# ambonvik/cimba

Measured on NVIDIA H100. Metric: M/M/1 simulated events/sec (FEL pops/s), higher is better.
Workload: dtype f64

## Files before the change

cimba_b200/csrc/mm1_fast.cuh:

```cuda
#pragma once

#include "engine.cuh"
#include "queue_model.cuh"
#include "rng.cuh"

namespace cimba_b200 {

#ifndef MM1_PARK_MASK
#define MM1_PARK_MASK 7u
#endif
#ifndef MM1_COLD_BATCH
#define MM1_COLD_BATCH 4
#endif

__device__ __forceinline__ void sts_f64(uint32_t addr, double v)
{
    asm volatile("st.shared.f64 [%0], %1;" :: "r"(addr), "d"(v) : "memory");
}

__device__ __forceinline__ double lds_f64(uint32_t addr)
{
    double v;
    asm volatile("ld.shared.f64 %0, [%1];" : "=d"(v) : "r"(addr) : "memory");
    return v;
}

__device__ __forceinline__ uint32_t pack_key(uint32_t counter, uint32_t action)
{
    return (counter << 2) | action;
}

template <bool TRACE>
__global__ void __launch_bounds__(QUEUE_BLOCK)
mm1_kernel(const QueueArgs a)
{
    __shared__ double exp_x[256];
    __shared__ double ring_smem[QUEUE_WINDOW * QUEUE_BLOCK];

    for (unsigned i = threadIdx.x; i < 256u; i += blockDim.x) {
        exp_x[i] = zig::zig_exp_x[i];
    }
    __syncthreads();

    constexpr unsigned FULL = 0xffffffffu;
    constexpr uint32_t WMASK = QUEUE_WINDOW - 1;
    constexpr uint32_t ROW = QUEUE_BLOCK * 8u;
    const double INF = __longlong_as_double(0x7ff0000000000000LL);
    const unsigned lane = threadIdx.x & 31u;
    const uint64_t gtid = (uint64_t)blockIdx.x * blockDim.x + threadIdx.x;
    uint64_t trial;
    bool alive;
    if (a.mapping == 32) {
        trial = gtid >> 5;
        alive = (lane == 0u) && (trial < a.num_trials);
    }
    else {
        trial = gtid;
        alive = trial < a.num_trials;
    }

    Sfc64 rng;
    rng.a = rng.b = rng.c = rng.d = 0u;
    double t_arr = INF, t_srv = INF;
    uint32_t k_arr = 0u, k_srv = 0u;
    uint32_t issued = 0u;
    double now = 0.0, stamp = 0.0, sum_wait = 0.0;
    double arr_mean = 1.0, srv_mean = 1.0;
    uint32_t produced = 0u, served = 0u, dropped = 0u, status = TRIAL_OK, longest = 0u;
    const uint32_t quota = (uint32_t)a.num_objects;
    uint32_t win = (uint32_t)__cvta_generic_to_shared(&ring_smem[threadIdx.x]);
    uint32_t tab = (uint32_t)__cvta_generic_to_shared(&exp_x[0]);
    __shared__ double scratch_smem[QUEUE_BLOCK];
    uint32_t scratch = (uint32_t)__cvta_generic_to_shared(&scratch_smem[threadIdx.x]);
    asm volatile("" : "+r"(win), "+r"(tab), "+r"(scratch));
    double *const spill = (a.spill_cap && alive) ? a.spill + trial * a.spill_cap : nullptr;
    const uint32_t spill_mask = a.spill_cap - 1u;

    uint64_t u_next = 0u;
    double e_next = 0.0;
    uint32_t pops = 0u;

    if (alive) {
        arr_mean = a.arr_mean[trial];
        srv_mean = a.srv_mean[trial];
        rng.seed(fmix64(a.master_seed, a.first_trial + trial));
        t_arr = 0.0; k_arr = pack_key(1u, ACT_START);
        t_srv = 0.0; k_srv = pack_key(2u, ACT_START);
        issued = 2u;
        u_next = rng.next();
        e_next = __dmul_rn(lds_f64(tab + ((uint32_t)u_next & 0xffu) * 8u), __ull2double_rn(u_next));
    }

    uint32_t flags = alive ? 1u : 0u;
    uint32_t step = 0u;

    while (__any_sync(FULL, flags & 1u)) {
        const bool go0 = (flags & 3u) == 1u;
        const bool first_arr = (t_arr < t_srv) | ((t_arr == t_srv) & (k_arr < k_srv));
        const uint32_t key = first_arr ? k_arr : k_srv;
        const uint32_t act = key & 3u;
        const bool go = go0 & (key != 0u);
        const bool done = go0 & (key == 0u);
        const bool is_arr = go & first_arr;
        const bool is_srv = go & !first_arr;
        const bool wake = act == ACT_WAKE_TIME;
        if (TRACE) {
            if (go && pops < a.trace_cap) {
                a.trace_key[trial * a.trace_cap + pops] = key >> 2;
                a.trace_time[trial * a.trace_cap + pops] = first_arr ? t_arr : t_srv;
            }
            pops += go ? 1u : 0u;
        }
        if (go) now = first_arr ? t_arr : t_srv;

        const uint32_t q_len = produced - served;
        const bool put = is_arr & wake;
        const bool put_far = put & (q_len >= (uint32_t)QUEUE_WINDOW);
        sts_f64((put & !put_far) ? win + (produced & WMASK) * ROW : scratch, now);
        if (put_far) {
            if (spill != nullptr && q_len - QUEUE_WINDOW <= spill_mask) {
                spill[produced & spill_mask] = now;
            }
            else {
                status |= TRIAL_ERR_QUEUE_OVERFLOW;
                dropped++;
                served++;
            }
        }
        if (put) produced++;
        longest = max(longest, produced - served);
        const bool ring_bell = put & (k_srv == 0u);
        if (ring_bell) {
            issued++;
            t_srv = now;
            k_srv = pack_key(issued, ACT_WAKE_RESOURCE);
        }

        const bool finished = is_srv & wake;
        const double new_sum = __dadd_rn(sum_wait, __dsub_rn(now, stamp));
        if (finished) sum_wait = new_sum;
        const bool take = is_srv & (produced != served);
        const uint32_t head_slot = win + (served & WMASK) * ROW;
        const double head_stamp = lds_f64(head_slot);
        if (take) stamp = head_stamp;
        if (take & (produced - served > (uint32_t)QUEUE_WINDOW)) {
            sts_f64(head_slot, spill[(served + QUEUE_WINDOW) & spill_mask]);
        }
        if (take) served++;

        const bool draw = take | (is_arr & (produced < quota));
        const bool hot = Sfc64::exp_is_hot(u_next);
        const bool push = draw & hot;
        const double when = __dadd_rn(now, __dmul_rn(is_arr ? arr_mean : srv_mean, e_next));
        if (push) issued++;
        const double t_new = push ? when : INF;
        const uint32_t k_new = push ? pack_key(issued, ACT_WAKE_TIME) : 0u;
        if (is_arr) { t_arr = t_new; k_arr = k_new; }
        if (is_srv) { t_srv = t_new; k_srv = k_new; }
        if (draw & !hot) flags = is_arr ? 7u : 3u;
        if (push) {
            u_next = rng.next();
            e_next = __dmul_rn(lds_f64(tab + ((uint32_t)u_next & 0xffu) * 8u), __ull2double_rn(u_next));
        }

        if (done) {
            flags = 0u;
            if (a.events)    a.events[trial] = issued;
            if (a.objects)   a.objects[trial] = served - dropped;
            if (a.t_end)     a.t_end[trial] = now;
            if (a.sum_wait)  a.sum_wait[trial] = sum_wait;
            if (a.status)    a.status[trial] = status | (issued > 0x3ffffff0u ? TRIAL_ERR_KEY_OVERFLOW : 0u);
            if (a.max_queue) a.max_queue[trial] = longest;
        }
        if ((++step & MM1_PARK_MASK) != 0u) {
            continue;
        }
        const unsigned pm = __ballot_sync(FULL, flags & 2u);
        if (pm != 0u) {
            const unsigned am = __ballot_sync(FULL, flags & 1u);
            if (__popc(pm) >= MM1_COLD_BATCH || pm == am) {
                if (flags & 2u) {
                    const bool parked_is_arr = (flags & 4u) != 0u;
                    const double mean = parked_is_arr ? arr_mean : srv_mean;
                    const double at = __dadd_rn(now, __dmul_rn(mean, rng.exp_cold(u_next)));
                    issued++;
                    if (parked_is_arr) { t_arr = at; k_arr = pack_key(issued, ACT_WAKE_TIME); }
                    else               { t_srv = at; k_srv = pack_key(issued, ACT_WAKE_TIME); }
                    flags = 1u;
                    u_next = rng.next();
                    e_next = __dmul_rn(lds_f64(tab + ((uint32_t)u_next & 0xffu) * 8u), __ull2double_rn(u_next));
                }
            }
        }
    }
    if (a.diag != nullptr && lane == 0u) {
        atomicAdd(a.diag, (unsigned long long)step);
        atomicAdd(a.diag + 1, 1ull);
    }
}

}
```

cimba_b200/csrc/rng.cuh:

```cuda
#pragma once

#include <cstdint>
#ifndef CMB_HOST_BUILD
#include <cuda_runtime.h>
#endif

#include "glibc_exp.cuh"
#include "zig_tables.cuh"

namespace cimba_b200 {

__host__ __device__ __forceinline__ uint64_t fmix64(uint64_t seed, uint64_t nonce)
{
    uint64_t h = seed + nonce;
    h ^= h >> 33;
    h *= 0xff51afd7ed558ccdULL;
    h ^= h >> 33;
    h *= 0xc4ceb9fe1a85ec53ULL;
    h ^= h >> 33;
    return h;
}

struct ZigHot {
    double exp_x[256];
    double nor_x[256];
};

__device__ __forceinline__ void stage_zig_hot(ZigHot &hot, bool want_normal)
{
    for (unsigned i = threadIdx.x; i < 256u; i += blockDim.x) {
        hot.exp_x[i] = zig::zig_exp_x[i];
        hot.nor_x[i] = want_normal ? zig::zig_nor_x[i] : 0.0;
    }
}

__device__ __noinline__ double zig_exp(double x)
{
    return glibc_exp(x);
}

constexpr double TWO_POW_64 = 18446744073709551616.0;
constexpr double TWO_POW_63 = 9223372036854775808.0;
constexpr double TWO_POW_M53 = 1.1102230246251565404e-16;

struct Sfc64 {
    uint64_t a, b, c, d;

    __device__ __forceinline__ uint64_t next()
    {
        const uint64_t out = a + b + d++;
        a = b ^ (b >> 11);
#if !defined(SFC64_NO_IMAD) && !defined(CMB_HOST_BUILD)
        {
            uint32_t lo, hi;
            asm("mov.b64 {%0, %1}, %2;" : "=r"(lo), "=r"(hi) : "l"(c));
            uint64_t w;
            asm("mul.wide.u32 %0, %1, 9;" : "=l"(w) : "r"(lo));
            uint32_t wl, wh;
            asm("mov.b64 {%0, %1}, %2;" : "=r"(wl), "=r"(wh) : "l"(w));
            asm("mad.lo.u32 %0, %1, 9, %2;" : "=r"(wh) : "r"(hi), "r"(wh));
            asm("mov.b64 %0, {%1, %2};" : "=l"(b) : "r"(wl), "r"(wh));
        }
#else
        b = c + (c << 3);
#endif
        c = ((c << 24) | (c >> 40)) + out;
        return out;
    }

    __device__ __forceinline__ void rewind()
    {
        const uint64_t pc = b * 0x8e38e38e38e38e39ULL;
        uint64_t pb = a;
        pb ^= pb >> 11;
        pb ^= pb >> 22;
        pb ^= pb >> 44;
        const uint64_t out = c - ((pc << 24) | (pc >> 40));
        d -= 1u;
        a = out - pb - d;
        b = pb;
        c = pc;
    }

    __device__ __forceinline__ void seed(uint64_t s)
    {
        uint64_t w[4];
#pragma unroll
        for (int i = 0; i < 4; i++) {
            uint64_t z = (s += 0x9e3779b97f4a7c15ULL);
            z = (z ^ (z >> 30)) * 0xbf58476d1ce4e5b9ULL;
            z = (z ^ (z >> 27)) * 0x94d049bb133111ebULL;
            w[i] = z ^ (z >> 31);
        }
        a = w[0];
        b = w[1];
        c = w[2];
        d = w[3];
#pragma unroll 1
        for (int i = 0; i < 20; i++) {
            (void)next();
        }
    }

    __device__ __forceinline__ double uniform01()
    {
        return __dmul_rn(__ull2double_rn(next() >> 11), TWO_POW_M53);
    }

    __device__ __forceinline__ double uniform(double lo, double hi)
    {
        return __dadd_rn(lo, __dmul_rn(__dsub_rn(hi, lo), uniform01()));
    }

    __device__ __forceinline__ unsigned bernoulli(double p)
    {
        return uniform01() <= p ? 1u : 0u;
    }

    __device__ __forceinline__ long long dice(long long lo, long long hi)
    {
        const double x = __dmul_rn(__ll2double_rn(hi - lo + 1), uniform01());
        return (long long)floor(__dadd_rn(__ll2double_rn(lo), x));
    }


    static __device__ __forceinline__ bool exp_is_hot(uint64_t u)
    {
        return (unsigned)(u & 0xffu) <= ZIG_EXP_MAX;
    }

    static __device__ __forceinline__ double exp_hot(const ZigHot &hot, uint64_t u)
    {
        return __dmul_rn(hot.exp_x[u & 0xffu], __ull2double_rn(u));
    }

    __device__ __forceinline__ double exp_cold(uint64_t ux)
    {
        double shift = 0.0;
        for (;;) {
            uint64_t uy = next();
            unsigned j = (unsigned)(uy & 0xffu);
            if (next() >= zig::zig_exp_prob[j]) {
                j = zig::zig_exp_alias[j];
            }
            if (j > 0u) {
                const double xj = zig::zig_exp_x[j];
                const double dx = __dsub_rn(zig::zig_exp_x[j - 1u], xj);
                for (;;) {
                    if (uy > (UINT64_MAX - ux)) {
                        uy = UINT64_MAX - uy;
                        ux = UINT64_MAX - ux;
                    }
                    const uint64_t gap = (UINT64_MAX - ux) - uy;
                    const double x = __dadd_rn(__dmul_rn(xj, TWO_POW_64),
                                               __dmul_rn(dx, __ull2double_rn(ux)));
                    if (gap >= zig::zig_exp_concavity[j]) {
                        return __dadd_rn(x, shift);
                    }
                    const double y0 = zig::zig_exp_y[j - 1u];
                    const double y = __dadd_rn(__dmul_rn(y0, TWO_POW_64),
                                               __dmul_rn(__dsub_rn(zig::zig_exp_y[j], y0),
                                                         __ull2double_rn(uy)));
                    if (y <= zig_exp(-x)) {
                        return __dadd_rn(x, shift);
                    }
                    uy = next();
                    ux = next();
                }
            }
            shift = __dadd_rn(shift, ZIG_EXP_TAIL);
            ux = next();
            const unsigned i = (unsigned)(ux & 0xffu);
            if (i <= ZIG_EXP_MAX) {
                return __dadd_rn(__dmul_rn(zig::zig_exp_x[i], __ull2double_rn(ux)), shift);
            }
        }
    }

    __device__ __forceinline__ double std_exponential(const ZigHot &hot)
    {
        const uint64_t u = next();
        return exp_is_hot(u) ? exp_hot(hot, u) : exp_cold(u);
    }

    __device__ __forceinline__ double std_exponential_global()
    {
        const uint64_t u = next();
        return exp_is_hot(u) ? __dmul_rn(zig::zig_exp_x[u & 0xffu], __ull2double_rn(u)) : exp_cold(u);
    }

    __device__ __forceinline__ double exponential(const ZigHot &hot, double mean)
    {
        return __dmul_rn(mean, std_exponential(hot));
    }

    __device__ __forceinline__ double erlang(const ZigHot &hot, unsigned k, double m)
    {
        double x = 0.0;
        for (unsigned i = 0u; i < k; i++) {
            x = __dadd_rn(x, exponential(hot, m));
        }
        return x;
    }


    __device__ __forceinline__ int64_t draw63()
    {
        return (int64_t)(next() & (uint64_t)INT64_MAX);
    }

    static __device__ __forceinline__ double nor_x_of(unsigned j, int64_t ix)
    {
        const double xj = zig::zig_nor_x[j];
        return __dadd_rn(__dmul_rn(xj, TWO_POW_63),
                         __dmul_rn(__dsub_rn(zig::zig_nor_x[j - 1u], xj), __ll2double_rn(ix)));
    }

    static __device__ __forceinline__ double nor_y_of(unsigned j, int64_t iy)
    {
        const double y0 = zig::zig_nor_y[j - 1u];
        return __dadd_rn(__dmul_rn(y0, TWO_POW_63),
                         __dmul_rn(__dsub_rn(zig::zig_nor_y[j], y0),
                                   __ull2double_rn((uint64_t)iy)));
    }

    static __device__ __forceinline__ double nor_pdf_scaled(double x)
    {
        return zig_exp(__dmul_rn(__dmul_rn(-0.5, x), x));
    }

    __device__ __forceinline__ double nor_cold(const ZigHot &hot, int64_t ix)
    {
        const double sign = (ix < 0) ? -1.0 : 1.0;
        ix &= INT64_MAX;
        int64_t iy = draw63();
        unsigned j = (unsigned)(iy & 0xff);
        if (ix >= zig::zig_nor_prob[j]) {
            j = zig::zig_nor_alias[j];
        }
        if (j > ZIG_NOR_INFLECTION) {
            for (;;) {
                const double x = nor_x_of(j, ix);
                const int64_t gap = (INT64_MAX - ix) - iy;
                if (gap >= 0) {
                    return __dmul_rn(sign, x);
                }
                if (gap + zig::zig_nor_convexity[j] >= 0) {
                    if (nor_y_of(j, iy) < nor_pdf_scaled(x)) {
                        return __dmul_rn(sign, x);
                    }
                }
                ix = draw63();
                iy = draw63();
            }
        }
        else if (j == 0u) {
            double x, z;
            do {
                x = __dmul_rn(ZIG_NOR_INV_TAIL, exponential(hot, 1.0));
                z = exponential(hot, 1.0);
            } while (__dmul_rn(2.0, z) <= __dmul_rn(x, x));
            return __dmul_rn(sign, __dadd_rn(x, ZIG_NOR_TAIL));
        }
        else if (j < ZIG_NOR_INFLECTION) {
            for (;;) {
                if (iy > INT64_MAX - ix) {
                    iy = INT64_MAX - iy;
                    ix = INT64_MAX - ix;
                }
                const double x = nor_x_of(j, ix);
                const int64_t gap = (INT64_MAX - ix) - iy;
                if (gap >= zig::zig_nor_concavity[j]) {
                    return __dmul_rn(sign, x);
                }
                if (nor_y_of(j, iy) <= nor_pdf_scaled(x)) {
                    return __dmul_rn(sign, x);
                }
                ix = draw63();
                iy = draw63();
            }
        }
        else {
            for (;;) {
                const double x = nor_x_of(j, ix);
                const int64_t gap = (INT64_MAX - ix) - iy;
                if (gap >= zig::zig_nor_concavity[j]) {
                    return __dmul_rn(sign, x);
                }
                if (gap + zig::zig_nor_convexity[j] > 0) {
                    if (nor_y_of(j, iy) < nor_pdf_scaled(x)) {
                        return __dmul_rn(sign, x);
                    }
                }
                ix = draw63();
                iy = draw63();
            }
        }
    }

    __device__ __forceinline__ double std_normal(const ZigHot &hot)
    {
        const int64_t ix = (int64_t)next();
        const unsigned i = (unsigned)(ix & 0xff);
        return (i <= ZIG_NOR_MAX) ? __dmul_rn(hot.nor_x[i], __ll2double_rn(ix))
                                  : nor_cold(hot, ix);
    }

    __device__ __forceinline__ double normal(const ZigHot &hot, double mu, double sigma)
    {
        return __dadd_rn(mu, __dmul_rn(sigma, std_normal(hot)));
    }
};

}
```

Measured before the change: 132.3 billion.

## Unroll two events per warp-vote iteration and route RNG shifts through IMAD

```diff
diff --git a/cimba_b200/csrc/mm1_fast.cuh b/cimba_b200/csrc/mm1_fast.cuh
--- a/cimba_b200/csrc/mm1_fast.cuh
+++ b/cimba_b200/csrc/mm1_fast.cuh
@@ -11,6 +11,9 @@
 #endif
 #ifndef MM1_COLD_BATCH
 #define MM1_COLD_BATCH 4
+#endif
+#ifndef MM1_STEPS
+#define MM1_STEPS 2
 #endif
 
 __device__ __forceinline__ void sts_f64(uint32_t addr, double v)
@@ -78,7 +81,13 @@
 
     uint64_t u_next = 0u;
     double e_next = 0.0;
+    uint32_t off_next = 0u;
     uint32_t pops = 0u;
+    const auto refill = [&]() {
+        u_next = rng.next_imad();
+        off_next = imad_hi(imad_lo((uint32_t)u_next, IMAD_K2P24, 0u), IMAD_K2P11, 0u);
+        e_next = __dmul_rn(lds_f64(tab + off_next), __ull2double_rn(u_next));
+    };
 
     if (alive) {
         arr_mean = a.arr_mean[trial];
@@ -87,23 +96,21 @@
         t_arr = 0.0; k_arr = pack_key(1u, ACT_START);
         t_srv = 0.0; k_srv = pack_key(2u, ACT_START);
         issued = 2u;
-        u_next = rng.next();
-        e_next = __dmul_rn(lds_f64(tab + ((uint32_t)u_next & 0xffu) * 8u), __ull2double_rn(u_next));
+        refill();
     }
 
     uint32_t flags = alive ? 1u : 0u;
     uint32_t step = 0u;
 
-    while (__any_sync(FULL, flags & 1u)) {
-        const bool go0 = (flags & 3u) == 1u;
+    const auto event_step = [&]() {
+        const bool go0 = flags == 1u;
         const bool first_arr = (t_arr < t_srv) | ((t_arr == t_srv) & (k_arr < k_srv));
         const uint32_t key = first_arr ? k_arr : k_srv;
-        const uint32_t act = key & 3u;
         const bool go = go0 & (key != 0u);
-        const bool done = go0 & (key == 0u);
+        if (go0 & (key == 0u)) flags = 0u;
         const bool is_arr = go & first_arr;
         const bool is_srv = go & !first_arr;
-        const bool wake = act == ACT_WAKE_TIME;
+        const bool wake = (key & 3u) == ACT_WAKE_TIME;
         if (TRACE) {
             if (go && pops < a.trace_cap) {
                 a.trace_key[trial * a.trace_cap + pops] = key >> 2;
@@ -113,43 +120,31 @@
         }
         if (go) now = first_arr ? t_arr : t_srv;
 
-        const uint32_t q_len = produced - served;
+        const uint32_t p0 = produced, s0 = served;
+        const uint32_t q_len = p0 - s0;
         const bool put = is_arr & wake;
         const bool put_far = put & (q_len >= (uint32_t)QUEUE_WINDOW);
-        sts_f64((put & !put_far) ? win + (produced & WMASK) * ROW : scratch, now);
-        if (put_far) {
-            if (spill != nullptr && q_len - QUEUE_WINDOW <= spill_mask) {
-                spill[produced & spill_mask] = now;
-            }
-            else {
-                status |= TRIAL_ERR_QUEUE_OVERFLOW;
-                dropped++;
-                served++;
-            }
-        }
+        sts_f64((put & !put_far) ? win + (p0 & WMASK) * ROW : scratch, now);
         if (put) produced++;
-        longest = max(longest, produced - served);
-        const bool ring_bell = put & (k_srv == 0u);
-        if (ring_bell) {
+        if (put & (k_srv == 0u)) {
             issued++;
             t_srv = now;
             k_srv = pack_key(issued, ACT_WAKE_RESOURCE);
         }
 
-        const bool finished = is_srv & wake;
         const double new_sum = __dadd_rn(sum_wait, __dsub_rn(now, stamp));
-        if (finished) sum_wait = new_sum;
-        const bool take = is_srv & (produced != served);
-        const uint32_t head_slot = win + (served & WMASK) * ROW;
+        if (is_srv & wake) sum_wait = new_sum;
+        const bool take = is_srv & (q_len != 0u);
+        const uint32_t head_slot = win + (s0 & WMASK) * ROW;
         const double head_stamp = lds_f64(head_slot);
-        if (take) stamp = head_stamp;
-        if (take & (produced - served > (uint32_t)QUEUE_WINDOW)) {
-            sts_f64(head_slot, spill[(served + QUEUE_WINDOW) & spill_mask]);
-        }
-        if (take) served++;
+        if (take) {
+            stamp = head_stamp;
+            served++;
+        }
+        const bool refill_far = take & (q_len > (uint32_t)QUEUE_WINDOW);
 
         const bool draw = take | (is_arr & (produced < quota));
-        const bool hot = Sfc64::exp_is_hot(u_next);
+        const bool hot = off_next <= ZIG_EXP_MAX * 8u;
         const bool push = draw & hot;
         const double when = __dadd_rn(now, __dmul_rn(is_arr ? arr_mean : srv_mean, e_next));
         if (push) issued++;
@@ -158,21 +153,31 @@
         if (is_arr) { t_arr = t_new; k_arr = k_new; }
         if (is_srv) { t_srv = t_new; k_srv = k_new; }
         if (draw & !hot) flags = is_arr ? 7u : 3u;
-        if (push) {
-            u_next = rng.next();
-            e_next = __dmul_rn(lds_f64(tab + ((uint32_t)u_next & 0xffu) * 8u), __ull2double_rn(u_next));
-        }
-
-        if (done) {
-            flags = 0u;
-            if (a.events)    a.events[trial] = issued;
-            if (a.objects)   a.objects[trial] = served - dropped;
-            if (a.t_end)     a.t_end[trial] = now;
-            if (a.sum_wait)  a.sum_wait[trial] = sum_wait;
-            if (a.status)    a.status[trial] = status | (issued > 0x3ffffff0u ? TRIAL_ERR_KEY_OVERFLOW : 0u);
-            if (a.max_queue) a.max_queue[trial] = longest;
-        }
-        if ((++step & MM1_PARK_MASK) != 0u) {
+        if (push) refill();
+
+        if (put_far | refill_far) {
+            if (refill_far) {
+                sts_f64(head_slot, spill[(s0 + QUEUE_WINDOW) & spill_mask]);
+            }
+            else if (spill != nullptr && q_len - QUEUE_WINDOW <= spill_mask) {
+                spill[p0 & spill_mask] = now;
+            }
+            else {
+                status |= TRIAL_ERR_QUEUE_OVERFLOW;
+                dropped++;
+                served++;
+            }
+        }
+        longest = max(longest, produced - served);
+    };
+
+    while (__any_sync(FULL, flags & 1u)) {
+#pragma unroll
+        for (int i = 0; i < MM1_STEPS; i++) {
+            event_step();
+        }
+        step += MM1_STEPS;
+        if ((step & MM1_PARK_MASK) != 0u) {
             continue;
         }
         const unsigned pm = __ballot_sync(FULL, flags & 2u);
@@ -187,11 +192,18 @@
                     if (parked_is_arr) { t_arr = at; k_arr = pack_key(issued, ACT_WAKE_TIME); }
                     else               { t_srv = at; k_srv = pack_key(issued, ACT_WAKE_TIME); }
                     flags = 1u;
-                    u_next = rng.next();
-                    e_next = __dmul_rn(lds_f64(tab + ((uint32_t)u_next & 0xffu) * 8u), __ull2double_rn(u_next));
+                    refill();
                 }
             }
         }
+    }
+    if (alive) {
+        if (a.events)    a.events[trial] = issued;
+        if (a.objects)   a.objects[trial] = served - dropped;
+        if (a.t_end)     a.t_end[trial] = now;
+        if (a.sum_wait)  a.sum_wait[trial] = sum_wait;
+        if (a.status)    a.status[trial] = status | (issued > 0x3ffffff0u ? TRIAL_ERR_KEY_OVERFLOW : 0u);
+        if (a.max_queue) a.max_queue[trial] = longest;
     }
     if (a.diag != nullptr && lane == 0u) {
         atomicAdd(a.diag, (unsigned long long)step);
diff --git a/cimba_b200/csrc/rng.cuh b/cimba_b200/csrc/rng.cuh
--- a/cimba_b200/csrc/rng.cuh
+++ b/cimba_b200/csrc/rng.cuh
@@ -42,6 +42,46 @@
 constexpr double TWO_POW_64 = 18446744073709551616.0;
 constexpr double TWO_POW_63 = 9223372036854775808.0;
 constexpr double TWO_POW_M53 = 1.1102230246251565404e-16;
+
+#ifndef CMB_HOST_BUILD
+static __constant__ uint32_t imad_k[3] = {1u << 21, 1u << 24, 1u << 11};
+#define IMAD_K2P21 imad_k[0]
+#define IMAD_K2P24 imad_k[1]
+#define IMAD_K2P11 imad_k[2]
+
+__device__ __forceinline__ uint64_t u64_of(uint32_t lo, uint32_t hi)
+{
+    uint64_t r;
+    asm("mov.b64 %0, {%1, %2};" : "=l"(r) : "r"(lo), "r"(hi));
+    return r;
+}
+
+__device__ __forceinline__ void u32_of(uint64_t v, uint32_t &lo, uint32_t &hi)
+{
+    asm("mov.b64 {%0, %1}, %2;" : "=r"(lo), "=r"(hi) : "l"(v));
+}
+
+__device__ __forceinline__ uint64_t imad_wide(uint32_t x, uint32_t y, uint64_t z)
+{
+    uint64_t r;
+    asm("mad.wide.u32 %0, %1, %2, %3;" : "=l"(r) : "r"(x), "r"(y), "l"(z));
+    return r;
+}
+
+__device__ __forceinline__ uint32_t imad_lo(uint32_t x, uint32_t y, uint32_t z)
+{
+    uint32_t r;
+    asm("mad.lo.u32 %0, %1, %2, %3;" : "=r"(r) : "r"(x), "r"(y), "r"(z));
+    return r;
+}
+
+__device__ __forceinline__ uint32_t imad_hi(uint32_t x, uint32_t y, uint32_t z)
+{
+    uint32_t r;
+    asm("mad.hi.u32 %0, %1, %2, %3;" : "=r"(r) : "r"(x), "r"(y), "r"(z));
+    return r;
+}
+#endif
 
 struct Sfc64 {
     uint64_t a, b, c, d;
@@ -68,6 +108,34 @@
         return out;
     }
 
+    __device__ __forceinline__ uint64_t next_imad()
+    {
+#if !defined(SFC64_NO_IMAD) && !defined(CMB_HOST_BUILD)
+        const uint64_t out = a + b + d++;
+        uint32_t bl, bh, cl, ch;
+        u32_of(b, bl, bh);
+        u32_of(c, cl, ch);
+        {
+            uint32_t wl, wh;
+            u32_of(imad_wide(bh, IMAD_K2P21, 0ull), wl, wh);
+            a = u64_of(bl ^ imad_hi(bl, IMAD_K2P21, 0u) ^ wl, bh ^ wh);
+        }
+        {
+            uint32_t wl, wh;
+            u32_of(imad_wide(cl, 9u, 0ull), wl, wh);
+            b = u64_of(wl, imad_lo(ch, 9u, wh));
+        }
+        {
+            uint32_t wl, wh;
+            u32_of(imad_wide(ch, IMAD_K2P24, 0ull), wl, wh);
+            c = imad_wide(cl, IMAD_K2P24, 0ull) + u64_of(wh, wl) + out;
+        }
+        return out;
+#else
+        return next();
+#endif
+    }
+
     __device__ __forceinline__ void rewind()
     {
         const uint64_t pc = b * 0x8e38e38e38e38e39ULL;
```

Result: faster. 138.0 billion (median of 6 runs) (+4.3%).
